# RL-VIG/LibContinual

Hardware: AMD Instinct MI355X
Metric: images/sec/node (task-0 epoch), CIFAR-100 B50-5x10 (higher is better)
Workload: dtype bf16; 1 GPU; lwf_resnet18_b50_task0; method=LWF, backbone=resnet18, per_gpu_batch=256, global_batch=256, image=3x32x32, parallelism=dp1, optimizer=fused SGD

## Files before the change

include/clhip.h:

```cpp
#ifndef CLHIP_H
#define CLHIP_H

#include <stddef.h>
#include <stdint.h>

#ifdef __cplusplus
extern "C" {
#endif

#define CLHIP_OK 0
#define CLHIP_EINVAL (-1)
#define CLHIP_EHIP (-2)
#define CLHIP_ENOMEM (-3)

#define CLHIP_BF16 0
#define CLHIP_F32 1

const char* clhip_last_error(void);
int clhip_version(void);

int clhip_nchw_to_nhwc(const float* x, void* y, int N, int C, int H, int W, int Cpad, int dtype, void* stream);
int clhip_nhwc_to_nchw(const void* y, float* x, int N, int C, int H, int W, int dtype, void* stream);

int clhip_conv_weight_prep(const float* w, void* w_fwd, void* w_dg, int K, int taps, int Creal, int Cpad,
// ... 225 lines not shown
    void* relu_mask;
} clhip_bn_res_input;
int clhip_conv_fwd_acc_bn_res_input(const void* z_in, const clhip_bn_input* bn , const clhip_bn_res_input* rs , const void* w_fwd, void* z,
                                    double* stat_acc, int replicas, int N, int H, int W, int C, int K, int ksize, int stride, int pad, int dtype,
                                    void* stream);
int clhip_conv_bn_input_wt_supported(int N, int H, int W, int C, int K, int ksize, int stride, int pad, int dtype);
int clhip_conv_fwd_acc_bn_input_wt(const void* z_in, const clhip_bn_input* bn , const clhip_bn_res_input* rs , const void* w_fwd, void* z,
                                   double* stat_acc, int replicas, int N, int H, int W, int C, int K, int ksize, int stride, int pad, int dtype,
                                   void* stream);
#define CLHIP_CONV_STEM7 1
#define CLHIP_CONV_STEM 2
#define CLHIP_CONV_CONV64 3
#define CLHIP_CONV_CONV16 4
#define CLHIP_CONV_CONV8 5
#define CLHIP_CONV_CONV5 6
#define CLHIP_CONV_CONV9 7
#define CLHIP_CONV_CONV4 8
#define CLHIP_CONV_CONV3 9
#define CLHIP_CONV_CONV2 10
#define CLHIP_CONV_V1 11
#define CLHIP_CONV_SHORTCUT 12
#define CLHIP_CONV_WGRAD_STEM7 13
#define CLHIP_CONV_WGRAD_STEM 14
#define CLHIP_CONV_WGRAD64 15
#define CLHIP_CONV_WGRAD4 16
#define CLHIP_CONV_WGRAD3 17
#define CLHIP_CONV_WGRAD16 18
#define CLHIP_CONV_WGRAD32 19
#define CLHIP_CONV_WGRAD2_DET 20
#define CLHIP_CONV_WGRAD2_ATOMIC 21
#define CLHIP_CONV_WGRAD_V1 22
#define CLHIP_CONV_WGRAD_V1_NO_TR 23
int clhip_conv_route(int op, int form, int N, int H, int W, int C, int Creal, int K, int ksize, int stride, int pad, int dtype);
int clhip_conv_dgrad_wgrad_bn_input(const void* x_z, const float* x_coef, const void* dz, const void* w_dg, void* dx, int accumulate, float* dw,
                                    void* ws, const float* mean, const float* invstd, double* acc , int replicas, int N, int H, int W,
                                    int C, int Creal, int K, int ksize, int stride, int pad, int dtype, void* stream);

int clhip_conv_dgrad_pair_supported(int N, int H, int W, int C, int K, int dtype);
size_t clhip_conv_dgrad_pair_packed_bytes(int C, int K);
int clhip_conv_dgrad_pair_pack(const void* w_dg, const void* w_sc_dg , void* packed, int C, int K, int dtype, void* stream);
int clhip_conv_dgrad_pair(const void* dz, const void* w_packed, const void* dz_sc , void* dx, int accumulate, int N, int H,
                          int W, int C, int K, int dtype, void* stream);

int clhip_conv_dgrad_pair_bn_reduce_supported(int N, int H, int W, int C, int K, int dtype);
int clhip_conv_dgrad_pair_bn_reduce(const void* dz, const void* w_packed, const void* dz_sc , void* dx, int accumulate, const void* z_prod,
                                    const void* y_prod , const float* mean, const float* invstd, double* acc, int replicas, int N, int H,
                                    int W, int C, int K, int dtype, void* stream);
int clhip_conv_wgrad_pair_supported(int N, int H, int W, int C, int K, int dtype);
int clhip_conv_fwd_acc_pair_supported(int N, int H, int W, int C, int K, int dtype);
int clhip_conv_fwd_acc_pair(const void* x, const void* w_fwd, const void* w_sc_fwd, void* z, void* z_sc, double* stat_acc, int replicas,
                            double* stat_acc_sc, int replicas_sc, int N, int H, int W, int C, int K, int dtype, void* stream);
int clhip_conv_wgrad_pair(const void* x, const void* dz, const void* dz_sc, float* dw, float* dw_sc, void* ws, void* ws_sc, int N, int H, int W,
                          int C, int K, int dtype, void* stream);

int clhip_config(const char* key, const char* value);
const char* clhip_config_get(const char* key);
void clhip_gemm8_config(int mode);
void clhip_wgrad4_config(int target_workgroups);
int clhip_attn_fwd(const void* qkv, void* out, float* lse, int B, int N, int H, int D, int dtype, void* stream);
int clhip_attn_bwd(const void* qkv, const void* out, const float* lse, const void* dout, void* dqkv, float* dsum_ws, int B, int N,
                   int H, int D, int dtype, void* stream);
int clhip_attn_prefix_fwd(const void* qkv, const void* pk, const void* pv, void* out, float* lse, int B, int N, int Lp, int H, int D, int dtype, void* stream);
int clhip_attn_prefix_bwd(const void* qkv, const void* pk, const void* pv, const void* out, const float* lse, const void* dout, void* dqkv, float* dpk,
                          float* dpv, float* dsum_ws, int B, int N, int Lp, int H, int D, int dtype, void* stream);
size_t clhip_coda_ws_bytes(int layers, int B, int s, int f);
int clhip_coda_fwd(int layers, const float* q, const float* const* K, const float* const* A, const float* const* P, void* const* ek, void* const* ev, float* c,
// ... 130 lines not shown
```

libcontinual_amd/_lib.py:

```python
import ctypes as C
import os
import re
import subprocess

_HERE = os.path.dirname(os.path.abspath(__file__))
LIB_PATH = os.path.join(_HERE, "libclhip.so")
HEADER_PATH = os.path.join(os.path.dirname(_HERE), "include", "clhip.h")

BF16, F32 = 0, 1
(CONV_STEM7, CONV_STEM, CONV_CONV64, CONV_CONV16, CONV_CONV8, CONV_CONV5, CONV_CONV9, CONV_CONV4, CONV_CONV3, CONV_CONV2, CONV_V1, CONV_SHORTCUT, CONV_WGRAD_STEM7,
 CONV_WGRAD_STEM, CONV_WGRAD64, CONV_WGRAD4, CONV_WGRAD3, CONV_WGRAD16, CONV_WGRAD32, CONV_WGRAD2_DET, CONV_WGRAD2_ATOMIC, CONV_WGRAD_V1, CONV_WGRAD_V1_NO_TR) = range(1, 24)


class ClhipError(RuntimeError):
    pass


class UnitDesc(C.Structure):
    _fields_ = [("cin", C.c_int32), ("cout", C.c_int32), ("ksize", C.c_int32), ("stride", C.c_int32), ("pad", C.c_int32),
                ("src", C.c_int32), ("res", C.c_int32), ("relu", C.c_int32),
                ("w_off", C.c_int64), ("gamma_off", C.c_int64), ("beta_off", C.c_int64),
                ("rm_off", C.c_int64), ("rv_off", C.c_int64)]


# ... 108 lines not shown
    "clhip_ce_slice": (_i, [_p, _p, _i, _i, _i, _i, _i, _f, _p, _i, _p, _i, _p, _p, _p]),
    "clhip_ce_window": (_i, [_p, _p, _i, _i, _i, _i, _i, _i, _f, _p, _i, _p, _i, _p, _p, _p]),
    "clhip_kd_loss": (_i, [_p, _i, _p, _i, _i, _i, _f, _f, _p, _i, _p, _i, _p]),
    "clhip_cosine_linear_fwd": (_i, [_p, _p, _p, _p, _p, _i, _i, _i, _p]),
    "clhip_cosine_linear_bwd": (_i, [_p, _p, _p, _p, _p, _p, _p, _p, _i, _i, _i, _i, _p]),
    "clhip_cos_embed_loss": (_i, [_p, _p, _i, _i, _f, _p, _i, _p, _i, _p]),
    "clhip_margin_rank_loss": (_i, [_p, _p, _i, _i, _i, _i, _f, _f, _p, _i, _p, _i, _p, _p]),
    "clhip_ewc_penalty": (_i, [_p, _p, _p, _l, _f, _p, _i, _p]),
    "clhip_ewc_grad": (_i, [_p, _p, _p, _p, _l, _f, _p, _p]),
    "clhip_ewc_penalty_multi": (_i, [_i, _p, _p, _p, _p, _f, _p, _i, _p]),
    "clhip_ewc_grad_multi": (_i, [_i, _p, _p, _p, _p, _p, _f, _p, _p]),
    "clhip_fisher_accum": (_i, [_p, _p, _l, _f, _p]),
    "clhip_fisher_merge": (_i, [_p, _p, _l, _f, _p]),
    "clhip_sgd_step": (_i, [_p, _p, _p, _l, _f, _f, _f, _f, _p, _p, _f, _p]),
    "clhip_sgd_step_multi": (_i, [_i, _p, _p, _p, _p, _f, _f, _f, _f, _p]),
    "clhip_sgd_step_multi_zero": (_i, [_i, _p, _p, _p, _p, _f, _f, _f, _f, C.c_uint, _p]),
    "clhip_adam_step": (_i, [_p, _p, _p, _p, _l, _f, _f, _f, _f, _f, _f, _i, _p]),
    "clhip_sq_norm": (_i, [_p, _l, _p, _i, _p]),
    "clhip_scale": (_i, [_p, _l, _f, _p]),
    "clhip_scale_dev": (_i, [_p, _p, _l, _f, _p, _p]),
    "clhip_sigma_scale_fwd": (_i, [_p, _p, _p, _l, _p]),
    "clhip_sigma_scale_bwd": (_i, [_p, _p, _p, _p, _p, _i, _l, _p]),
    "clhip_l2_normalize_rows": (_i, [_p, _p, _i, _i, _p]),
    "clhip_ncm_classify": (_i, [_p, _p, _i, _i, _i, _p, _p]),
    "clhip_herding_select": (_i, [_p, _i, _i, _i, _p, _p, _p]),
    "clhip_herding_select_batched": (_i, [_p, _p, _i, _i, _i, _i, _p, _p, _p]),
    "clhip_augment_crop_flip": (_i, [_p, _p, _p, _p, _p, _i, _i, _i, _i, _i, C.POINTER(C.c_float), C.POINTER(C.c_float), _p]),
    "clhip_augment_rrc_flip": (_i, [_p, _p, _p, _p, _i, _i, _i, _i, C.POINTER(C.c_float), C.POINTER(C.c_float), _p]),
    "clhip_augment_rrc_aa_ws_bytes": (_sz, [_i, _i, _i]),
    "clhip_augment_rrc_aa": (_i, [_p, _p, _p, _p, _p, _p, _p, _i, _i, _i, _i, _i, C.POINTER(C.c_float), C.POINTER(C.c_float), _p]),
    "clhip_gemm_nt": (_i, [_p, _p, _p, _p, _p, _p] + [_i] * 10 + [_p]),
    "clhip_gemm_nt_route": (_i, [_i] * 9 + [C.POINTER(C.c_int), _i]),
    "clhip_conv_route": (_i, [_i] * 12),
    "clhip_config": (_i, [C.c_char_p, C.c_char_p]),
    "clhip_config_get": (C.c_char_p, [C.c_char_p]),
    "clhip_conv_bn_input_wt_supported": (_i, [_i] * 9),
    "clhip_conv_fwd_acc_bn_input_wt": (_i, [_p, _p, _p, _p, _p, _p, _i] + [_i] * 9 + [_p]),
    "clhip_gram_accum_batched": (_i, [_p, C.c_size_t, _i, _p, _i, _i, _i, _p]),
    "clhip_gemm8_config": (None, [_i]),
    "clhip_wgrad4_config": (None, [_i]),
    "clhip_attn_fwd": (_i, [_p, _p, _p, _i, _i, _i, _i, _i, _p]),
    "clhip_attn_bwd": (_i, [_p, _p, _p, _p, _p, _p, _i, _i, _i, _i, _i, _p]),
    "clhip_attn_prefix_fwd": (_i, [_p, _p, _p, _p, _p, _i, _i, _i, _i, _i, _i, _p]),
    "clhip_attn_prefix_bwd": (_i, [_p] * 10 + [_i] * 6 + [_p]),
    "clhip_coda_ws_bytes": (_sz, [_i, _i, _i, _i]),
    "clhip_coda_fwd": (_i, [_i, _p, _p, _p, _p, _p, _p, _p, _i, _i, _i, _i, _i, _i, _p]),
    "clhip_coda_bwd": (_i, [_i] + [_p] * 11 + [_i] * 6 + [_p]),
    "clhip_dual_fwd": (_i, [_i, _i] + [_p] * 9 + [_i] * 8 + [_p]),
    "clhip_dual_bwd": (_i, [_i, _i] + [_p] * 8 + [_i] * 6 + [_p]),
    "clhip_ln_fwd": (_i, [_p, _p, _p, _p, _p, _p, _i, _i, _f, _i, _p]),
    "clhip_ln_bwd": (_i, [_p, _p, _p, _p, _p, _p, _i, _i, _i, _p]),
    "clhip_ln_pool_fwd": (_i, [_p, _p, _p, _p, _i, _i, _i, _i, _f, _i, _p]),
    "clhip_ln_pool_bwd": (_i, [_p, _p, _p, _p, _i, _i, _i, _i, _f, _i, _p]),
    "clhip_patchify": (_i, [_p, _p, _i, _i, _i, _i, _p]),
    "clhip_vit_assemble": (_i, [_p, _p, _p, _p, _p, _i, _i, _i, _i, _i, _p]),
    "clhip_vit_prompt_grad": (_i, [_p, _p, _i, _i, _i, _i, _i, _p]),
    "clhip_weight_prep2": (_i, [_p, _p, _p, _i, _i, _p, _p, _p, _p, _i, _i, _p]),
    "clhip_lora_qkv_refresh": (_i, [_i, _p, _p, _p, _p, _p, _p, _p, _i, _i, _i, _p]),
    "clhip_lora_merge": (_i, [_p, _p, _p, _p, _p, _i, _i, _p]),
    "clhip_lora_grad_ws_bytes": (_sz, [_i, _i, _i]),
    "clhip_lora_acat": (_i, [_p, _p, _p, _i, _i, _i, _p]),
    "clhip_lora_grad": (_i, [_p, _p, _p, _p, _p, _p, _p, _p, _i, _i, _i, _i, _p]),
    "clhip_gram_accum": (_i, [_p, _p, _i, _i, _i, _p]),
    "clhip_l2p_select": (_i, [_p, _p, _p, _i, _i, _i, _i, _i, _p, _p, _p, _p, _p, _p]),
    "clhip_l2p_scatter": (_i, [_p, _p, _p, _i, _i, _i, _i, _p]),
    "clhip_vit_create": (_p, [C.POINTER(VitDesc), _i]),
# ... 82 lines not shown
```

libcontinual_amd/csrc/api.hip:

```cpp
#include <map>
#include <utility>
#include <vector>
#include <mutex>
#include <string>
#include <string.h>
#include <stdio.h>
#include <stdlib.h>

#include "kernels.h"

static thread_local char g_err[512] = "";

void clhip_set_error(const char* fmt, ...) {
    va_list ap;
    va_start(ap, fmt);
    vsnprintf(g_err, sizeof(g_err), fmt, ap);
    va_end(ap);
}

extern "C" const char* clhip_last_error(void) { return g_err; }
extern "C" int clhip_version(void) { return 103; }

namespace {
const char* const kKeys[] = {
    "ATTN_GENERIC", "ATTN_BWD", "BN_FUSE", "BN_FUSE_MAX_M", "BN_MASK_BITS", "BN_MASK_FROM_Y", "BN_PARTIALS", "CE_ROWS", "CE_ONE_WG", "LINEAR_BWD_SPLIT", "CONV3G", "CONV4", "CONV_V1",
    "GEMM_NO_SPLIT", "GEMM_TAIL", "NO_CONV16", "NO_CONV3", "NO_PARITY_DGRAD", "NO_SHORTCUT", "NO_STEM", "PREP_NARROW", "WGRAD4",
    "WGRAD_NO_TR", "WGRAD2_ATOMIC", "WGRAD_DEFER", "WGRAD_DEFER_SIDE", "BWD_FUSED", "WGRAD_STREAM", "BRANCH_STREAM", "WGRAD_ALWAYS_QUEUE", "SIDE_PRIO", "EVENT_FLAGS", "EVENT_RECORD", "CONV5", "CONV6", "WGRAD16_PARTS", "WGRAD32_IPG", "WGRAD64_IPG", "WGRAD64_IPI2", "CONV64", "CONV64_BM", "CONV64_FWD", "CONV6_PAIR", "CONV7", "CONV7_TPW", "WGRAD7", "FWD7", "PAIR_BN_FUSE", "POOL_BN_FUSE", "BN_INPUT", "BN_INPUT_WT", "BN_RES_INPUT", "BN_GRAD", "BN_GRAD_MINC", "BN_GRAD_RES", "CONV6_DEBUG", "BN_ONEPASS", "WGRAD5", "WGRAD32",
    "BN_ACC_CPT", "BN_BWD_ITERS", "CONV3_CFG", "CONV4_CFG", "CONV4_GRID", "GEMM_GROUP_M", "GEMM_MT", "IGEMM_TILE",
    "SHORTCUT_MIN_PIXELS", "STEM_GRID", "STEM_WGRAD_GRID", "WGRAD4_MIN_STEPS", "WGRAD4_MIN_TOTAL", "WGRAD_NET_GFLOP", "WGRAD_TARGET",
    "CONV5_MIN_TILES", "CONV5_GRID", "CONV64_MAX_W", "CONV64_MAX_M", "CONV8", "CONV8_MIN_TILES", "DZ_BUFFERS", "CONV8_GRID", "CONV8_OPT", "CONV8_BNR", "CONV9", "PLAN_SKIP", "WT_DEBUG", "EVAL_LAZY", "GEMM_SPLITK", "STREAM_PROBE", "STAGE_EVAL", "STAGE_TRAIN", "STAGE_TRAIN_BWD", "STAGE_TRACE", "STAGE_ENTRY", "STAGE_ENTRY_BWD", "STAGE_POOL", "STAGE_XCH3", "ADAPTER_TM",
    "CONV3_DEBUG", "WGRAD_DEBUG", "CONV4_FORCE_CFG", "CONV4_ENABLE", "CONV4_DEBUG", "CONV4_TRACE", "WGRAD4_TRACE", "CONV6_TRACE", "CONV8_TRACE", "CONV9_TRACE",
};
std::mutex g_stream_mu;
std::mutex g_cfg_mu;
std::map<std::string, const char*>& cfg_map() { static std::map<std::string, const char*> m; return m; }
bool known_key(const char* k) {
    for (const char* q : kKeys) if (strcmp(q, k) == 0) return true;
    return false;
}
}

namespace {
__global__ void stream_probe_spin_kernel(unsigned long long* out, long long ticks) {
    const unsigned long long t0 = wall_clock64();
    while ((long long)(wall_clock64() - t0) < ticks) __builtin_amdgcn_s_sleep(64);
    out[0] = wall_clock64();
}
__global__ void stream_probe_stamp_kernel(unsigned long long* out) { out[1] = wall_clock64(); }

struct SharedStreams {
    std::vector<hipStream_t> pool;
    std::map<std::pair<hipStream_t, int>, hipStream_t> chosen;
    hipStream_t low_prio = nullptr;
    unsigned long long* probe_buf = nullptr;
};
SharedStreams g_shared[16];

bool runs_beside(SharedStreams& S, hipStream_t a, hipStream_t b) {
// ... 111 lines not shown
```

libcontinual_amd/csrc/bn.hip:

```cpp
#include <stdlib.h>

#include <hip/hip_ext.h>

#include "kernels.h"

namespace {

__global__ __launch_bounds__(256) void bn_finalize_kernel(const float* __restrict__ part, int tiles, double invM, double unbias,
                                                          int C, const float* __restrict__ gamma, const float* __restrict__ beta,
                                                          float* rm, float* rv, float momentum, float eps, float* mean_o,
                                                          float* invstd_o, float* scale, float* shift) {
    const int lane = threadIdx.x & 63, wave = threadIdx.x >> 6;
    const int c = blockIdx.x * 4 + wave;
    if (c >= C) return;
    double s1 = 0.0, s2 = 0.0;
    for (int t = lane; t < tiles; t += 64) {
        s1 += (double)part[((size_t)t * 2 + 0) * C + c];
        s2 += (double)part[((size_t)t * 2 + 1) * C + c];
    }
#pragma unroll
    for (int o = 32; o > 0; o >>= 1) { s1 += __shfl_xor(s1, o, 64); s2 += __shfl_xor(s2, o, 64); }
    if (lane == 0) {
        double mean = s1 * invM;
        double var = s2 * invM - mean * mean;
// ... 193 lines not shown
}

template <typename T, bool RELU, int DRES>
__global__ __launch_bounds__(256) void bn_bwd_apply_kernel(const T* __restrict__ dy, const T* __restrict__ y,
                                                           const T* __restrict__ z, const float* __restrict__ mean,
                                                           const float* __restrict__ invstd, const float* __restrict__ gamma,
                                                           const float* __restrict__ coef, T* __restrict__ dz, T* __restrict__ dres,
                                                           int64_t nchunks, int C) {
    const int64_t stride = (int64_t)gridDim.x * blockDim.x;
    for (int64_t i = (int64_t)blockIdx.x * blockDim.x + threadIdx.x; i < nchunks; i += stride) {
        const int c0 = (int)((i * 8) % C);
        float g[8], yy[8], zz[8], o[8], rr[8];
        load8<T>(dy + i * 8, g);
        load8<T>(z + i * 8, zz);
        if (RELU) load8<T>(y + i * 8, yy);
        if (DRES == 2) load8<T>(dres + i * 8, rr);
#pragma unroll
        for (int e = 0; e < 8; ++e) {
            const int c = c0 + e;
            float gg = g[e];
            if (RELU) gg = yy[e] > 0.f ? gg : 0.f;
            const float is = invstd[c];
            const float xh = (zz[e] - mean[c]) * is;
            o[e] = gamma[c] * is * (gg - coef[c] - xh * coef[C + c]);
            g[e] = gg;
            if (DRES == 2) rr[e] += gg;
        }
        store8<T>(dz + i * 8, o);
        if (DRES == 1) store8<T>(dres + i * 8, g);
        if (DRES == 2) store8<T>(dres + i * 8, rr);
    }
}

template <typename T, bool RES, bool RELU>
__global__ __launch_bounds__(256) void bn_apply_train_kernel(const T* __restrict__ z, const double* __restrict__ acc, int rep, double invM, double unbias,
                                                             const float* __restrict__ gamma, const float* __restrict__ beta, float* rm, float* rv,
                                                             float momentum, float eps, float* __restrict__ mean_o, float* __restrict__ invstd_o,
                                                             const T* __restrict__ res, T* __restrict__ y, int64_t nchunks, int C,
                                                             unsigned char* __restrict__ relu_mask = nullptr) {
    extern __shared__ __attribute__((aligned(16))) float coefs[];
    __shared__ double sred[256];
    const bool narrow = 2 * C <= 128;
    if (narrow) replica_parts(acc, rep, C, sred);
    for (int c = threadIdx.x; c < C; c += 256) {
        const bool upd = blockIdx.x == 0 && rm != nullptr;
        const float rm_old = upd ? rm[c] : 0.f, rv_old = upd ? rv[c] : 0.f;
        double s1 = 0.0, s2 = 0.0;
        if (narrow) { for (int q = 0; q < 256 / (2 * C); ++q) { s1 += sred[q * 2 * C + c]; s2 += sred[q * 2 * C + C + c]; } }
        else sum_strided2(acc + c, acc + C + c, rep, 2 * (size_t)C, s1, s2);
        const double mean = s1 * invM;
        double var = s2 * invM - mean * mean;
        if (var < 0.0) var = 0.0;
        float istd;
        if constexpr (sizeof(T) == 4) istd = (float)(1.0 / sqrt(var + (double)eps));
        else istd = rsqrtf((float)var + eps);
        const float sc = gamma[c] * istd;
        coefs[c] = sc;
        coefs[C + c] = beta[c] - (float)mean * sc;
        if (blockIdx.x == 0) {
            mean_o[c] = (float)mean;
            invstd_o[c] = istd;
            if (rm != nullptr) {
                rm[c] = (1.f - momentum) * rm_old + momentum * (float)mean;
                rv[c] = (1.f - momentum) * rv_old + momentum * (float)(var * unbias);
            }
        }
    }
    __syncthreads();
    const int64_t stride = (int64_t)gridDim.x * blockDim.x;
    const int64_t i0 = (int64_t)blockIdx.x * blockDim.x + threadIdx.x;
    const int c0 = ((int)i0 & ((C >> 3) - 1)) * 8;
    float sc[8], sh[8];
#pragma unroll
    for (int e = 0; e < 8; ++e) { sc[e] = coefs[c0 + e]; sh[e] = coefs[C + c0 + e]; }
    constexpr int UN = 4;
    for (int64_t i = i0; i < nchunks; i += stride * UN) {
        float v[UN][8], r[UN][8];
#pragma unroll
        for (int u = 0; u < UN; ++u) {
            const int64_t iu = i + u * stride;
            if (iu < nchunks) { load8<T>(z + iu * 8, v[u]); if (RES) load8<T>(res + iu * 8, r[u]); }
        }
#pragma unroll
        for (int u = 0; u < UN; ++u) {
            const int64_t iu = i + u * stride;
            if (iu >= nchunks) break;
#pragma unroll
            for (int e = 0; e < 8; ++e) {
                float o = fmaf(v[u][e], sc[e], sh[e]);
                if (RES) o += r[u][e];
                if (RELU) o = fmaxf(o, 0.f);
                v[u][e] = o;
            }
            store8<T>(y + iu * 8, v[u]);
            if (RELU && relu_mask != nullptr) {
                unsigned m = 0;
#pragma unroll
                for (int e = 0; e < 8; ++e) m |= (stored_positive<T>(v[u][e]) ? 1u : 0u) << e;
                relu_mask[iu] = (unsigned char)m;
            }
        }
    }
}

template <typename T, int RELU, int DRES>
__global__ __launch_bounds__(256) void bn_bwd_apply_acc_kernel(const T* __restrict__ dy, const T* __restrict__ y, const T* __restrict__ z,
                                                               const float* __restrict__ mean, const float* __restrict__ invstd,
                                                               const float* __restrict__ gamma, const double* __restrict__ acc, int rep, double invM,
                                                               float* dgamma, float* dbeta, T* __restrict__ dz, T* __restrict__ dres,
                                                               int64_t nchunks, int C, const float* __restrict__ beta = nullptr) {
    extern __shared__ __attribute__((aligned(16))) float coefs[];
    __shared__ double sred[256];
    const bool narrow = 2 * C <= 128;
    if (narrow) replica_parts(acc, rep, C, sred);
    for (int c = threadIdx.x; c < C; c += 256) {
        const float db_old = blockIdx.x == 0 ? dbeta[c] : 0.f, dg_old = blockIdx.x == 0 ? dgamma[c] : 0.f;
        const float m = mean[c], is_c = invstd[c], gi_c = gamma[c] * is_c;
        const float sh_c = RELU == 2 ? beta[c] - m * gi_c : 0.f;
        double s1 = 0.0, s2 = 0.0;
        if (narrow) { for (int q = 0; q < 256 / (2 * C); ++q) { s1 += sred[q * 2 * C + c]; s2 += sred[q * 2 * C + C + c]; } }
        else sum_strided2(acc + c, acc + C + c, rep, 2 * (size_t)C, s1, s2);
        coefs[c] = (float)(s1 * invM);
        coefs[C + c] = (float)(s2 * invM);
        coefs[2 * C + c] = m;
        coefs[3 * C + c] = is_c;
        coefs[4 * C + c] = gi_c;
        coefs[5 * C + c] = sh_c;
        if (blockIdx.x == 0) { dbeta[c] = db_old + (float)s1; dgamma[c] = dg_old + (float)s2; }
    }
    __syncthreads();
    const int64_t stride = (int64_t)gridDim.x * blockDim.x;
    const int64_t i0 = (int64_t)blockIdx.x * blockDim.x + threadIdx.x;
    const int c0 = ((int)i0 & ((C >> 3) - 1)) * 8;
    float k0[8], k1[8], gi[8], mu[8], is[8], sh[8];
#pragma unroll
    for (int e = 0; e < 8; ++e) {
        k0[e] = coefs[c0 + e];
        k1[e] = coefs[C + c0 + e];
        mu[e] = coefs[2 * C + c0 + e];
        is[e] = coefs[3 * C + c0 + e];
        gi[e] = coefs[4 * C + c0 + e];
        if (RELU == 2) sh[e] = coefs[5 * C + c0 + e];
    }
    constexpr int UN = sizeof(T) == 2 ? 4 : 2;
    for (int64_t i = i0; i < nchunks; i += stride * UN) {
        float g[UN][8], yy[UN][8], zz[UN][8], rr[UN][8];
        unsigned mk[UN];
#pragma unroll
        for (int u = 0; u < UN; ++u) {
            mk[u] = 0;
            const int64_t iu = i + u * stride;
            if (iu < nchunks) {
                load8<T>(dy + iu * 8, g[u]);
                load8<T>(z + iu * 8, zz[u]);
                if (RELU == 1) load8<T>(y + iu * 8, yy[u]);
                if (RELU == 3) mk[u] = reinterpret_cast<const unsigned char*>(y)[iu];
                if (DRES == 2) load8<T>(dres + iu * 8, rr[u]);
            }
        }
#pragma unroll
        for (int u = 0; u < UN; ++u) {
            const int64_t iu = i + u * stride;
            if (iu >= nchunks) break;
            float o[8];
#pragma unroll
            for (int e = 0; e < 8; ++e) {
                float gg = g[u][e];
                if (RELU == 1) gg = yy[u][e] > 0.f ? gg : 0.f;
                if (RELU == 2) gg = stored_positive<T>(fmaf(zz[u][e], gi[e], sh[e])) ? gg : 0.f;
                if (RELU == 3) gg = (mk[u] >> e) & 1u ? gg : 0.f;
                const float xh = (zz[u][e] - mu[e]) * is[e];
                o[e] = gi[e] * (gg - k0[e] - xh * k1[e]);
                g[u][e] = gg;
                if (DRES == 2) rr[u][e] += gg;
            }
            store8<T>(dz + iu * 8, o);
            if (DRES == 1) store8<T>(dres + iu * 8, g[u]);
            if (DRES == 2) store8<T>(dres + iu * 8, rr[u]);
        }
    }
}

int bn_bwd_blocks(int64_t M, int C) {
    int cpr = C >> 3;
    int rpi = 256 / cpr;
    int64_t g = (M + rpi - 1) / rpi;
    static const int forced = clhip_cfg("BN_BWD_ITERS") ? atoi(clhip_cfg("BN_BWD_ITERS")) : 0;
    int64_t iters = forced > 0 ? forced : g / 128;
    if (iters < 1) iters = 1;
    if (iters > 8) iters = 8;
    g = (g + iters - 1) / iters;
    if (g > 1024) g = 1024;
    if (g < 1) g = 1;
    return (int)g;
}

// ... 586 lines not shown
```

libcontinual_amd/csrc/conv2.hip:

```cpp
#include <stdlib.h>

#include "kernels.h"

namespace {

constexpr int BK2 = 64;

struct ConvParams2 {
    const void* src;
    const void* wt;
    void* dst;
    float* stats;
    double* stat_acc;
    int stat_rep;
    int N, Hs, Ws, Cs, log2Cs, Hd, Wd, Cd, ksize, stride, pad, accumulate;
    int M, K;
    int cls_tiles;
};

template <typename T> struct Chunk2;
template <> struct Chunk2<bf16_t> { uint4 a; };
template <> struct Chunk2<float> { uint4 a, b; };

template <typename T> __device__ __forceinline__ Chunk2<T> zero2() {
    Chunk2<T> c;
    if constexpr (sizeof(T) == 2) { c.a = make_uint4(0, 0, 0, 0); }
    else { c.a = make_uint4(0, 0, 0, 0); c.b = make_uint4(0, 0, 0, 0); }
    return c;
}
template <typename T> __device__ __forceinline__ Chunk2<T> gload2(const T* p) {
    Chunk2<T> c;
    if constexpr (sizeof(T) == 2) { c.a = *reinterpret_cast<const uint4*>(p); }
    else { c.a = *reinterpret_cast<const uint4*>(p); c.b = *reinterpret_cast<const uint4*>(p + 4); }
// ... 290 lines not shown
    dim3 grid((p.M + BM - 1) / BM, (p.Cd + BN - 1) / BN);
    ConvParams2 q = p;
    if (q.cls_tiles > 0) {
        q.cls_tiles = (q.M / 4 + BM - 1) / BM;
        grid.x = 4 * q.cls_tiles;
    }
    hipLaunchKernelGGL(kern, grid, dim3(256), lds, st, q);
    CLHIP_LAUNCH_CHECK();
    return CLHIP_OK;
}

template <typename T, int MODE>
int launch2(const ConvParams2& p, hipStream_t st) {
    TileCfg t = pick_tile(p.cls_tiles > 0 ? p.M / 4 : p.M, p.Cd);
    if (t.bn == 128) {
        if (t.bm == 128) return launch_cfg<T, 2, 2, 4, 4, MODE>(p, st);
        return launch_cfg<T, 1, 4, 4, 2, MODE>(p, st);
    }
    if (t.bn == 64) {
        if (t.bm == 256) return launch_cfg<T, 4, 1, 4, 4, MODE>(p, st);
        if (t.bm == 128) return launch_cfg<T, 4, 1, 2, 4, MODE>(p, st);
        return launch_cfg<T, 4, 1, 1, 4, MODE>(p, st);
    }
    if (t.bn == 32) {
        if (t.bm == 256) return launch_cfg<T, 4, 1, 4, 2, MODE>(p, st);
        if (t.bm == 128) return launch_cfg<T, 4, 1, 2, 2, MODE>(p, st);
        return launch_cfg<T, 4, 1, 1, 2, MODE>(p, st);
    }
    if (t.bm == 256) return launch_cfg<T, 4, 1, 4, 1, MODE>(p, st);
    if (t.bm == 128) return launch_cfg<T, 4, 1, 2, 1, MODE>(p, st);
    return launch_cfg<T, 4, 1, 1, 1, MODE>(p, st);
}

}

int clhip_conv2_tiles_m(int M, int Cd) { return (M + pick_tile(M, Cd).bm - 1) / pick_tile(M, Cd).bm; }

int clhip_conv2_launch(const void* src, const void* wt, void* dst, float* stats, double* stat_acc, int stat_rep, int N, int Hs, int Ws, int Cs, int Hd, int Wd,
                       int Cd, int ksize, int stride, int pad, int accumulate, int mode, int dtype, hipStream_t st) {
    ConvParams2 p;
    p.src = src; p.wt = wt; p.dst = dst; p.stats = stats; p.stat_acc = stat_acc; p.stat_rep = stat_rep > 0 ? stat_rep : 1;
    p.N = N; p.Hs = Hs; p.Ws = Ws; p.Cs = Cs; p.log2Cs = ilog2_exact(Cs); p.Hd = Hd; p.Wd = Wd; p.Cd = Cd;
    p.ksize = ksize; p.stride = stride; p.pad = pad; p.accumulate = accumulate;
    p.M = N * Hd * Wd; p.K = ksize * ksize * Cs;
    static const bool nocls = clhip_cfg("NO_PARITY_DGRAD") != nullptr;
    p.cls_tiles = (!nocls && mode == 1 && stride == 2 && ksize == 3 && Cs >= 32 && p.log2Cs >= 0 && (Hd % 2 == 0) && (Wd % 2 == 0)) ? 1 : 0;
    if (dtype == CLHIP_BF16) return mode == 0 ? launch2<bf16_t, 0>(p, st) : launch2<bf16_t, 1>(p, st);
    return mode == 0 ? launch2<float, 0>(p, st) : launch2<float, 1>(p, st);
}

namespace {

#ifdef CLHIP_ABLATION
#define DBGW2(p) ((p).debug)
#else
#define DBGW2(p) 0
#endif

struct WgradParams2 {
    const void* x; const void* dz; float* dw;
    int N, H, W, C, log2C, Creal, Ho, Wo, lgHo, lgWo, K, ksize, stride, pad;
    int M, J, pix_per_split, debug;
    float* slab;
    int64_t slab_stride;
};

template <typename T>
__device__ __forceinline__ Chunk2<T> lds_ld_tr(const char* tile, int pitch, int pix0, int col0, int lane) {
    const int fr = lane & 15, fg = lane >> 4;
    Chunk2<T> c;
    if constexpr (sizeof(T) == 2) {
        const char* a0 = tile + (pix0 + fg * 8 + (fr >> 2)) * pitch + (col0 + (fr & 3) * 4) * 2;
// ... 219 lines not shown
```

libcontinual_amd/trainer.py:

```python
import copy
import os
import sys
from time import time

import numpy as np
import torch
from torch.utils.data import DataLoader

from . import ops, parallel
from . import scheduler as sched
from .utils import AverageMeter, compute_bwt, compute_frgt, count_all_parameters, count_parameters, get_instance, init_seed, quiesce_gc

_OBSERVE_DOES_BACKWARD = ("L2P",)


_UNIT_GRADS = {}


def _backward(loss):
    if loss.is_cuda and loss.dim() == 0 and loss.dtype == torch.float32:
        one = _UNIT_GRADS.get(loss.device)
        if one is None:
            one = _UNIT_GRADS[loss.device] = torch.ones((), device=loss.device, dtype=torch.float32)
            ops.UNIT_GRAD_PTRS.add(one.data_ptr())
        torch.autograd.backward(loss, grad_tensors=one)
    else:
        loss.backward()


class GraphedStep:
    WARM, KEEP = 2, 4
    PROBE = 12
    _PLAN_SWITCHES = (b"BN_INPUT", b"BN_INPUT_WT", b"BN_RES_INPUT", b"BN_GRAD", b"BN_GRAD_RES", b"BN_FUSE", b"BRANCH_STREAM", b"WGRAD_STREAM", b"CONV6_PAIR",
                      b"STAGE_EVAL", b"EVAL_LAZY", b"STAGE_TRAIN", b"STAGE_TRAIN_BWD", b"STAGE_ENTRY", b"STAGE_POOL", b"STAGE_XCH3", b"GEMM8", b"GEMM_TAIL", b"ATTN_BWD")

    def __init__(self, model, optimizer, method_name, reducer=None):
        self.model, self.optimizer, self.method_name = model, optimizer, method_name
        self.reducer = reducer
        from .optim import _owner_of
        owners = {}
        for group in optimizer.param_groups:
            for p in group["params"]:
                o = _owner_of(p)
                if o is not None:
                    owners[id(o)] = o
        self.owners = list(owners.values())
        self.graphs = {}
        self.seen = {}
        self.stream = torch.cuda.Stream()
        self.choice = {}
        self._probe = {}
        self.disabled = False
        self.fallback_ok = True

    def _key(self, batch):
        shapes = tuple((k, tuple(v.shape), str(v.dtype)) for k, v in sorted(batch.items()) if torch.is_tensor(v))
        lrs = tuple((g.get("lr"), g.get("momentum"), g.get("weight_decay")) for g in self.optimizer.param_groups)
        from . import _lib
        L = _lib.lib()
        cfg = tuple(L.clhip_config_get(k) for k in self._PLAN_SWITCHES)
        red = self.reducer
        dp = None if red is None else (red.world, red.exchange, getattr(self.optimizer, "grad_scale", None))
        return shapes, lrs, self.model.training, cfg, dp

    def _step(self, batch):
        if self.method_name in _OBSERVE_DOES_BACKWARD:
            self.optimizer.zero_grad()
# ... 496 lines not shown
```

Before: 131,400 images/sec.

## Add pipelined LDS-direct stride-2 entry conv kernel and prefetch BN apply loads

Adds a specialized bf16 3x3 stride-2 downsampling convolution kernel for stage-entry layers. It uses buffer loads straight into LDS with a three-stage ring, MFMA accumulation and fused BN statistics, and is enabled by default under an ENTRY_S2 switch that is also registered as a plan switch. It also issues the first global loads in the BN apply forward and backward kernels before the coefficient reduction and syncthreads, so memory latency overlaps the reduction. The cost is extra register pressure and one more kernel variant; a launch counter is exported for observability.

```diff
diff --git a/include/clhip.h b/include/clhip.h
--- a/include/clhip.h
+++ b/include/clhip.h
@@ -281,6 +281,7 @@
 #define CLHIP_CONV_WGRAD_V1 22
 #define CLHIP_CONV_WGRAD_V1_NO_TR 23
 int clhip_conv_route(int op, int form, int N, int H, int W, int C, int Creal, int K, int ksize, int stride, int pad, int dtype);
+long long clhip_conv_entry_s2_launches(void);
 int clhip_conv_dgrad_wgrad_bn_input(const void* x_z, const float* x_coef, const void* dz, const void* w_dg, void* dx, int accumulate, float* dw,
                                     void* ws, const float* mean, const float* invstd, double* acc , int replicas, int N, int H, int W,
                                     int C, int Creal, int K, int ksize, int stride, int pad, int dtype, void* stream);
diff --git a/libcontinual_amd/_lib.py b/libcontinual_amd/_lib.py
--- a/libcontinual_amd/_lib.py
+++ b/libcontinual_amd/_lib.py
@@ -164,6 +164,7 @@
     "clhip_gemm_nt": (_i, [_p, _p, _p, _p, _p, _p] + [_i] * 10 + [_p]),
     "clhip_gemm_nt_route": (_i, [_i] * 9 + [C.POINTER(C.c_int), _i]),
     "clhip_conv_route": (_i, [_i] * 12),
+    "clhip_conv_entry_s2_launches": (C.c_longlong, []),
     "clhip_config": (_i, [C.c_char_p, C.c_char_p]),
     "clhip_config_get": (C.c_char_p, [C.c_char_p]),
     "clhip_conv_bn_input_wt_supported": (_i, [_i] * 9),
diff --git a/libcontinual_amd/csrc/api.hip b/libcontinual_amd/csrc/api.hip
--- a/libcontinual_amd/csrc/api.hip
+++ b/libcontinual_amd/csrc/api.hip
@@ -23,7 +23,7 @@
 
 namespace {
 const char* const kKeys[] = {
-    "ATTN_GENERIC", "ATTN_BWD", "BN_FUSE", "BN_FUSE_MAX_M", "BN_MASK_BITS", "BN_MASK_FROM_Y", "BN_PARTIALS", "CE_ROWS", "CE_ONE_WG", "LINEAR_BWD_SPLIT", "CONV3G", "CONV4", "CONV_V1",
+    "ATTN_GENERIC", "ATTN_BWD", "BN_FUSE", "BN_FUSE_MAX_M", "BN_MASK_BITS", "BN_MASK_FROM_Y", "BN_PARTIALS", "CE_ROWS", "CE_ONE_WG", "LINEAR_BWD_SPLIT", "CONV3G", "CONV4", "CONV_V1", "ENTRY_S2",
     "GEMM_NO_SPLIT", "GEMM_TAIL", "NO_CONV16", "NO_CONV3", "NO_PARITY_DGRAD", "NO_SHORTCUT", "NO_STEM", "PREP_NARROW", "WGRAD4",
     "WGRAD_NO_TR", "WGRAD2_ATOMIC", "WGRAD_DEFER", "WGRAD_DEFER_SIDE", "BWD_FUSED", "WGRAD_STREAM", "BRANCH_STREAM", "WGRAD_ALWAYS_QUEUE", "SIDE_PRIO", "EVENT_FLAGS", "EVENT_RECORD", "CONV5", "CONV6", "WGRAD16_PARTS", "WGRAD32_IPG", "WGRAD64_IPG", "WGRAD64_IPI2", "CONV64", "CONV64_BM", "CONV64_FWD", "CONV6_PAIR", "CONV7", "CONV7_TPW", "WGRAD7", "FWD7", "PAIR_BN_FUSE", "POOL_BN_FUSE", "BN_INPUT", "BN_INPUT_WT", "BN_RES_INPUT", "BN_GRAD", "BN_GRAD_MINC", "BN_GRAD_RES", "CONV6_DEBUG", "BN_ONEPASS", "WGRAD5", "WGRAD32",
     "BN_ACC_CPT", "BN_BWD_ITERS", "CONV3_CFG", "CONV4_CFG", "CONV4_GRID", "GEMM_GROUP_M", "GEMM_MT", "IGEMM_TILE",
diff --git a/libcontinual_amd/csrc/bn.hip b/libcontinual_amd/csrc/bn.hip
--- a/libcontinual_amd/csrc/bn.hip
+++ b/libcontinual_amd/csrc/bn.hip
@@ -249,6 +249,20 @@
     }
 }
 
+template <typename T> struct Raw8;
+template <> struct Raw8<bf16_t> { uint4 a; };
+template <> struct Raw8<float> { float4 a, b; };
+template <typename T> __device__ __forceinline__ Raw8<T> raw_load8(const T* p) {
+    Raw8<T> r;
+    if constexpr (sizeof(T) == 2) { r.a = *reinterpret_cast<const uint4*>(p); }
+    else { r.a = *reinterpret_cast<const float4*>(p); r.b = *reinterpret_cast<const float4*>(p + 4); }
+    return r;
+}
+template <typename T> __device__ __forceinline__ void raw_unpack8(const Raw8<T>& r, float (&v)[8]) {
+    if constexpr (sizeof(T) == 2) { unpack8(r.a, v); }
+    else { v[0] = r.a.x; v[1] = r.a.y; v[2] = r.a.z; v[3] = r.a.w; v[4] = r.b.x; v[5] = r.b.y; v[6] = r.b.z; v[7] = r.b.w; }
+}
+
 template <typename T, bool RES, bool RELU>
 __global__ __launch_bounds__(256) void bn_apply_train_kernel(const T* __restrict__ z, const double* __restrict__ acc, int rep, double invM, double unbias,
                                                              const float* __restrict__ gamma, const float* __restrict__ beta, float* rm, float* rv,
@@ -256,6 +270,15 @@
                                                              const T* __restrict__ res, T* __restrict__ y, int64_t nchunks, int C,
                                                              unsigned char* __restrict__ relu_mask = nullptr) {
     extern __shared__ __attribute__((aligned(16))) float coefs[];
+    constexpr int UN = 4;
+    const int64_t stride = (int64_t)gridDim.x * blockDim.x;
+    const int64_t i0 = (int64_t)blockIdx.x * blockDim.x + threadIdx.x;
+    Raw8<T> pv[UN], pr[UN];
+#pragma unroll
+    for (int u = 0; u < UN; ++u) {
+        const int64_t iu = i0 + u * stride;
+        if (iu < nchunks) { pv[u] = raw_load8<T>(z + iu * 8); if (RES) pr[u] = raw_load8<T>(res + iu * 8); }
+    }
     __shared__ double sred[256];
     const bool narrow = 2 * C <= 128;
     if (narrow) replica_parts(acc, rep, C, sred);
@@ -284,24 +307,25 @@
         }
     }
     __syncthreads();
-    const int64_t stride = (int64_t)gridDim.x * blockDim.x;
-    const int64_t i0 = (int64_t)blockIdx.x * blockDim.x + threadIdx.x;
     const int c0 = ((int)i0 & ((C >> 3) - 1)) * 8;
     float sc[8], sh[8];
 #pragma unroll
     for (int e = 0; e < 8; ++e) { sc[e] = coefs[c0 + e]; sh[e] = coefs[C + c0 + e]; }
-    constexpr int UN = 4;
     for (int64_t i = i0; i < nchunks; i += stride * UN) {
         float v[UN][8], r[UN][8];
-#pragma unroll
-        for (int u = 0; u < UN; ++u) {
-            const int64_t iu = i + u * stride;
-            if (iu < nchunks) { load8<T>(z + iu * 8, v[u]); if (RES) load8<T>(res + iu * 8, r[u]); }
+        if (i != i0) {
+#pragma unroll
+            for (int u = 0; u < UN; ++u) {
+                const int64_t iu = i + u * stride;
+                if (iu < nchunks) { pv[u] = raw_load8<T>(z + iu * 8); if (RES) pr[u] = raw_load8<T>(res + iu * 8); }
+            }
         }
 #pragma unroll
         for (int u = 0; u < UN; ++u) {
             const int64_t iu = i + u * stride;
             if (iu >= nchunks) break;
+            raw_unpack8<T>(pv[u], v[u]);
+            if (RES) raw_unpack8<T>(pr[u], r[u]);
 #pragma unroll
             for (int e = 0; e < 8; ++e) {
                 float o = fmaf(v[u][e], sc[e], sh[e]);
@@ -327,6 +351,26 @@
                                                                float* dgamma, float* dbeta, T* __restrict__ dz, T* __restrict__ dres,
                                                                int64_t nchunks, int C, const float* __restrict__ beta = nullptr) {
     extern __shared__ __attribute__((aligned(16))) float coefs[];
+    constexpr int UN = sizeof(T) == 2 ? 4 : 2;
+    const int64_t stride = (int64_t)gridDim.x * blockDim.x;
+    const int64_t i0 = (int64_t)blockIdx.x * blockDim.x + threadIdx.x;
+    Raw8<T> pg[UN], pz[UN], py[UN], pr[UN];
+    unsigned mk[UN];
+    auto issue = [&](int64_t i) {
+#pragma unroll
+        for (int u = 0; u < UN; ++u) {
+            mk[u] = 0;
+            const int64_t iu = i + u * stride;
+            if (iu < nchunks) {
+                pg[u] = raw_load8<T>(dy + iu * 8);
+                pz[u] = raw_load8<T>(z + iu * 8);
+                if (RELU == 1) py[u] = raw_load8<T>(y + iu * 8);
+                if (RELU == 3) mk[u] = reinterpret_cast<const unsigned char*>(y)[iu];
+                if (DRES == 2) pr[u] = raw_load8<T>(dres + iu * 8);
+            }
+        }
+    };
+    issue(i0);
     __shared__ double sred[256];
     const bool narrow = 2 * C <= 128;
     if (narrow) replica_parts(acc, rep, C, sred);
@@ -346,8 +390,6 @@
         if (blockIdx.x == 0) { dbeta[c] = db_old + (float)s1; dgamma[c] = dg_old + (float)s2; }
     }
     __syncthreads();
-    const int64_t stride = (int64_t)gridDim.x * blockDim.x;
-    const int64_t i0 = (int64_t)blockIdx.x * blockDim.x + threadIdx.x;
     const int c0 = ((int)i0 & ((C >> 3) - 1)) * 8;
     float k0[8], k1[8], gi[8], mu[8], is[8], sh[8];
 #pragma unroll
@@ -359,26 +401,17 @@
         gi[e] = coefs[4 * C + c0 + e];
         if (RELU == 2) sh[e] = coefs[5 * C + c0 + e];
     }
-    constexpr int UN = sizeof(T) == 2 ? 4 : 2;
     for (int64_t i = i0; i < nchunks; i += stride * UN) {
         float g[UN][8], yy[UN][8], zz[UN][8], rr[UN][8];
-        unsigned mk[UN];
-#pragma unroll
-        for (int u = 0; u < UN; ++u) {
-            mk[u] = 0;
-            const int64_t iu = i + u * stride;
-            if (iu < nchunks) {
-                load8<T>(dy + iu * 8, g[u]);
-                load8<T>(z + iu * 8, zz[u]);
-                if (RELU == 1) load8<T>(y + iu * 8, yy[u]);
-                if (RELU == 3) mk[u] = reinterpret_cast<const unsigned char*>(y)[iu];
-                if (DRES == 2) load8<T>(dres + iu * 8, rr[u]);
-            }
-        }
+        if (i != i0) issue(i);
 #pragma unroll
         for (int u = 0; u < UN; ++u) {
             const int64_t iu = i + u * stride;
             if (iu >= nchunks) break;
+            raw_unpack8<T>(pg[u], g[u]);
+            raw_unpack8<T>(pz[u], zz[u]);
+            if (RELU == 1) raw_unpack8<T>(py[u], yy[u]);
+            if (DRES == 2) raw_unpack8<T>(pr[u], rr[u]);
             float o[8];
 #pragma unroll
             for (int e = 0; e < 8; ++e) {
diff --git a/libcontinual_amd/csrc/conv2.hip b/libcontinual_amd/csrc/conv2.hip
--- a/libcontinual_amd/csrc/conv2.hip
+++ b/libcontinual_amd/csrc/conv2.hip
@@ -1,4 +1,6 @@
 #include <stdlib.h>
+
+#include <atomic>
 
 #include "kernels.h"
 
@@ -355,12 +357,234 @@
     return launch_cfg<T, 4, 1, 1, 1, MODE>(p, st);
 }
 
-}
+typedef __attribute__((address_space(3))) void lvoid_t;
+
+std::atomic<unsigned long long> g_entry_s2_launches{0};
+
+struct EntryS2Params {
+    const bf16_t* src;
+    const bf16_t* wt;
+    bf16_t* dst;
+    float* stats;
+    double* stat_acc;
+    int stat_rep;
+    int N, H, W, Cs, Cd, Hd, Wd, M;
+    int lgWd, lgHd, cpt_shift;
+};
+
+constexpr int ES_NST = 3;
+
+template <int N> __device__ __forceinline__ void es_wait_vm() { __builtin_amdgcn_s_waitcnt((N & 15) | 0x70 | 0xF00 | ((N >> 4) << 14)); }
+__device__ __forceinline__ void es_barrier() {
+    __builtin_amdgcn_s_waitcnt(0xC07F);
+    __builtin_amdgcn_s_barrier();
+    asm volatile("" ::: "memory");
+}
+
+template <int WM, int WN, int MT, int NT>
+__global__ __launch_bounds__(256) void conv_entry_s2_kernel(const EntryS2Params p) {
+    typedef bf16_t T;
+    constexpr int BM = WM * MT * 16, BN = WN * NT * 16;
+    constexpr int A_BYTES = BM * 128, STAGE = (BM + BN) * 128;
+    constexpr int AINST = BM / 8 / 4, BINST = BN / 8 / 4, WINST = AINST + BINST;
+    static_assert(WM * WN == 4 && AINST >= 1 && BINST >= 1 && AINST * 32 == BM && BINST * 32 == BN, "ring rows must divide among the four waves");
+    extern __shared__ __attribute__((aligned(16))) char smem[];
+    const int tid = threadIdx.x, lane = tid & 63;
+    const int wave = __builtin_amdgcn_readfirstlane(tid >> 6);
+    const int wm = wave / WN, wn = wave % WN;
+    const int m0 = blockIdx.x * BM, n0 = blockIdx.y * BN;
+    const int Cs = p.Cs, W = p.W, K9 = 9 * Cs;
+    constexpr int OOB = 0x40000000;
+
+    const int drow = lane >> 3, dslot = lane & 7;
+    int aoff[AINST], boff[BINST];
+    unsigned amask[AINST];
+#pragma unroll
+    for (int i = 0; i < AINST; ++i) {
+        const int row = (wave * AINST + i) * 8 + drow, pix = m0 + row;
+        aoff[i] = 0; amask[i] = 0;
+        if (pix < p.M) {
+            const int wo = pix & (p.Wd - 1), t = pix >> p.lgWd, ho = t & (p.Hd - 1), n = t >> p.lgHd;
+            const int h0 = 2 * ho - 1, w0 = 2 * wo - 1;
+            aoff[i] = (((n * p.H + h0) * W + w0) * Cs) * 2 + ((dslot ^ drow) << 4);
+            unsigned m = 0;
+#pragma unroll
+            for (int r = 0; r < 3; ++r)
+#pragma unroll
+                for (int s = 0; s < 3; ++s)
+                    if ((unsigned)(h0 + r) < (unsigned)p.H && (unsigned)(w0 + s) < (unsigned)W) m |= 1u << (3 * r + s);
+            amask[i] = m;
+        }
+    }
+#pragma unroll
+    for (int i = 0; i < BINST; ++i) {
+        const int row = (wave * BINST + i) * 8 + drow;
+        boff[i] = ((n0 + row) * K9) * 2 + ((dslot ^ drow) << 4);
+    }
+    const __amdgpu_buffer_rsrc_t srs = __builtin_amdgcn_make_buffer_rsrc(const_cast<bf16_t*>(p.src), 0, p.N * p.H * W * Cs * 2, 0x00020000);
+    const __amdgpu_buffer_rsrc_t wrs = __builtin_amdgcn_make_buffer_rsrc(const_cast<bf16_t*>(p.wt), 0, p.Cd * K9 * 2, 0x00020000);
+    auto issue = [&](int k, int stage) {
+        const int tap = k >> p.cpt_shift, chunk = k - (tap << p.cpt_shift);
+        const int r = tap / 3, s = tap - 3 * r;
+        const int tapoff = ((r * W + s) * Cs + chunk * 64) * 2;
+        const unsigned bit = 1u << tap;
+        char* l = smem + stage * STAGE;
+#if defined(__HIP_DEVICE_COMPILE__)
+#pragma unroll
+        for (int i = 0; i < AINST; ++i)
+            __builtin_amdgcn_raw_ptr_buffer_load_lds(srs, (lvoid_t*)(l + (wave * AINST + i) * 1024), 16, (amask[i] & bit) ? aoff[i] + tapoff : OOB, 0, 0, 0);
+#pragma unroll
+        for (int i = 0; i < BINST; ++i)
+            __builtin_amdgcn_raw_ptr_buffer_load_lds(wrs, (lvoid_t*)(l + A_BYTES + (wave * BINST + i) * 1024), 16, boff[i] + k * 128, 0, 0, 0);
+#else
+        (void)tapoff; (void)bit; (void)l;
+#endif
+    };
+
+    f32x4 acc[MT][NT];
+#pragma unroll
+    for (int i = 0; i < MT; ++i)
+#pragma unroll
+        for (int j = 0; j < NT; ++j) acc[i][j] = f32x4{0.f, 0.f, 0.f, 0.f};
+
+    const int fr = lane & 15, fg = lane >> 4;
+    const int nk = 9 << p.cpt_shift;
+    issue(0, 0);
+    issue(1, 1);
+#pragma unroll 1
+    for (int k0 = 0; k0 < nk; k0 += 3) {
+#pragma unroll
+        for (int s3 = 0; s3 < 3; ++s3) {
+            const int k = k0 + s3;
+            if (k + 1 < nk) es_wait_vm<WINST>(); else es_wait_vm<0>();
+            es_barrier();
+            if (k + 2 < nk) issue(k + 2, (s3 + 2) % 3);
+            const char* As = smem + s3 * STAGE;
+            const char* Bs = As + A_BYTES;
+#pragma unroll
+            for (int ks = 0; ks < 2; ++ks) {
+                bf16x8_t xf[MT], wf[NT];
+#pragma unroll
+                for (int i = 0; i < MT; ++i) xf[i] = *reinterpret_cast<const bf16x8_t*>(As + lds_off2<T>((wm * MT + i) * 16 + fr, ks * 4 + fg));
+#pragma unroll
+                for (int j = 0; j < NT; ++j) wf[j] = *reinterpret_cast<const bf16x8_t*>(Bs + lds_off2<T>((wn * NT + j) * 16 + fr, ks * 4 + fg));
+#pragma unroll
+                for (int i = 0; i < MT; ++i)
+#pragma unroll
+                    for (int j = 0; j < NT; ++j) acc[i][j] = __builtin_amdgcn_mfma_f32_16x16x32_bf16(wf[j], xf[i], acc[i][j], 0, 0, 0);
+            }
+        }
+    }
+
+#pragma unroll
+    for (int i = 0; i < MT; ++i) {
+        const int pix = m0 + (wm * MT + i) * 16 + fr;
+        if (pix < p.M) {
+#pragma unroll
+            for (int j = 0; j < NT; ++j) {
+                const int o = n0 + (wn * NT + j) * 16 + fg * 4;
+                uint2 u;
+                u.x = pack_bf16x2(acc[i][j][0], acc[i][j][1]);
+                u.y = pack_bf16x2(acc[i][j][2], acc[i][j][3]);
+                *reinterpret_cast<uint2*>(p.dst + (size_t)pix * p.Cd + o) = u;
+            }
+        }
+    }
+    if (p.stats == nullptr && p.stat_acc == nullptr) return;
+
+    es_barrier();
+    float* red = reinterpret_cast<float*>(smem);
+    float sv[8 * NT];
+#pragma unroll
+    for (int j = 0; j < NT; ++j)
+#pragma unroll
+        for (int e = 0; e < 4; ++e) {
+            float s1 = 0.f, s2 = 0.f;
+#pragma unroll
+            for (int i = 0; i < MT; ++i) { const float v = acc[i][j][e]; s1 += v; s2 = fmaf(v, v, s2); }
+            sv[j * 4 + e] = s1;
+            sv[4 * NT + j * 4 + e] = s2;
+        }
+    row16_sum_n(sv);
+    if (fr == 0) {
+#pragma unroll
+        for (int j = 0; j < NT; ++j) {
+            const int c = (wn * NT + j) * 16 + fg * 4;
+            *reinterpret_cast<float4*>(red + (wm * 2 + 0) * BN + c) = make_float4(sv[j * 4], sv[j * 4 + 1], sv[j * 4 + 2], sv[j * 4 + 3]);
+            *reinterpret_cast<float4*>(red + (wm * 2 + 1) * BN + c) = make_float4(sv[4 * NT + j * 4], sv[4 * NT + j * 4 + 1], sv[4 * NT + j * 4 + 2], sv[4 * NT + j * 4 + 3]);
+        }
+    }
+    es_barrier();
+    for (int idx = tid; idx < 2 * BN; idx += 256) {
+        const int which = idx / BN, c = idx - which * BN;
+        float t = 0.f;
+#pragma unroll
+        for (int w = 0; w < WM; ++w) t += red[(w * 2 + which) * BN + c];
+        if (p.stat_acc != nullptr) atomicAdd(p.stat_acc + ((size_t)(blockIdx.x & (p.stat_rep - 1)) * 2 + which) * p.Cd + n0 + c, (double)t);
+        else p.stats[((size_t)blockIdx.x * 2 + which) * p.Cd + n0 + c] = t;
+    }
+}
+
+bool entry_s2_domain(const void* stats, const double* stat_acc, int N, int Hs, int Ws, int Cs, int Hd, int Wd, int Cd, int ksize, int stride, int pad,
+                     int accumulate, int mode, int dtype) {
+    if (!(mode == 0 && dtype == CLHIP_BF16 && !(stats != nullptr && stat_acc != nullptr) && accumulate == 0)) return false;
+    if (!(ksize == 3 && stride == 2 && pad == 1 && Cd == 2 * Cs && (Cs == 64 || Cs == 128 || Cs == 256))) return false;
+    if (!(Hs == Ws && (Hs == 8 || Hs == 16 || Hs == 32) && Hd == Hs / 2 && Wd == Ws / 2 && N >= 1)) return false;
+    return (int64_t)N * Hs * Ws * Cs * 2 < ((int64_t)1 << 29);
+}
+
+template <int WM, int WN, int MT, int NT>
+int launch_entry_s2_cfg(const EntryS2Params& p, hipStream_t st) {
+    constexpr int BM = WM * MT * 16, BN = WN * NT * 16;
+    constexpr size_t lds = (size_t)ES_NST * (BM + BN) * 128;
+    static_assert(lds <= 160 * 1024 && lds >= WM * 2 * BN * sizeof(float), "LDS of one CU; the statistics scratch aliases the ring");
+    auto kern = conv_entry_s2_kernel<WM, WN, MT, NT>;
+    int dev = 0;
+    (void)hipGetDevice(&dev);
+    static bool attr_set[16] = {false};
+    if (dev < 0 || dev >= 16 || !attr_set[dev]) {
+        if (hipFuncSetAttribute(reinterpret_cast<const void*>(kern), hipFuncAttributeMaxDynamicSharedMemorySize, (int)lds) != hipSuccess) {
+            clhip_set_error("conv2 entry body: cannot reserve %zu bytes of LDS", lds);
+            return CLHIP_EHIP;
+        }
+        if (dev >= 0 && dev < 16) attr_set[dev] = true;
+    }
+    hipLaunchKernelGGL(kern, dim3((p.M + BM - 1) / BM, p.Cd / BN), dim3(256), lds, st, p);
+    CLHIP_LAUNCH_CHECK();
+    g_entry_s2_launches.fetch_add(1, std::memory_order_relaxed);
+    return CLHIP_OK;
+}
+
+int launch_entry_s2(const void* src, const void* wt, void* dst, float* stats, double* stat_acc, int stat_rep, int N, int Hs, int Ws, int Cs, int Hd, int Wd, int Cd,
+                    hipStream_t st, bool* launched) {
+    *launched = false;
+    const TileCfg t = pick_tile(N * Hd * Wd, Cd);
+    if (t.bn != 128 || t.bm != 64) return CLHIP_OK;
+    EntryS2Params p;
+    p.src = static_cast<const bf16_t*>(src); p.wt = static_cast<const bf16_t*>(wt); p.dst = static_cast<bf16_t*>(dst);
+    p.stats = stats; p.stat_acc = stat_acc; p.stat_rep = stat_rep > 0 ? stat_rep : 1;
+    p.N = N; p.H = Hs; p.W = Ws; p.Cs = Cs; p.Cd = Cd; p.Hd = Hd; p.Wd = Wd; p.M = N * Hd * Wd;
+    p.lgWd = ilog2_exact(Wd); p.lgHd = ilog2_exact(Hd); p.cpt_shift = ilog2_exact(Cs / 64);
+    *launched = true;
+    return launch_entry_s2_cfg<1, 4, 4, 2>(p, st);
+}
+
+}
+
+extern "C" long long clhip_conv_entry_s2_launches(void) { return (long long)g_entry_s2_launches.load(std::memory_order_relaxed); }
 
 int clhip_conv2_tiles_m(int M, int Cd) { return (M + pick_tile(M, Cd).bm - 1) / pick_tile(M, Cd).bm; }
 
 int clhip_conv2_launch(const void* src, const void* wt, void* dst, float* stats, double* stat_acc, int stat_rep, int N, int Hs, int Ws, int Cs, int Hd, int Wd,
                        int Cd, int ksize, int stride, int pad, int accumulate, int mode, int dtype, hipStream_t st) {
+    if (entry_s2_domain(stats, stat_acc, N, Hs, Ws, Cs, Hd, Wd, Cd, ksize, stride, pad, accumulate, mode, dtype)) {
+        const char* sw = clhip_cfg("ENTRY_S2");
+        if (sw == nullptr || atoi(sw) != 0) {
+            bool launched = false;
+            const int rc = launch_entry_s2(src, wt, dst, stats, stat_acc, stat_rep, N, Hs, Ws, Cs, Hd, Wd, Cd, st, &launched);
+            if (launched || rc != CLHIP_OK) return rc;
+        }
+    }
     ConvParams2 p;
     p.src = src; p.wt = wt; p.dst = dst; p.stats = stats; p.stat_acc = stat_acc; p.stat_rep = stat_rep > 0 ? stat_rep : 1;
     p.N = N; p.Hs = Hs; p.Ws = Ws; p.Cs = Cs; p.log2Cs = ilog2_exact(Cs); p.Hd = Hd; p.Wd = Wd; p.Cd = Cd;
diff --git a/libcontinual_amd/trainer.py b/libcontinual_amd/trainer.py
--- a/libcontinual_amd/trainer.py
+++ b/libcontinual_amd/trainer.py
@@ -32,7 +32,7 @@
     WARM, KEEP = 2, 4
     PROBE = 12
     _PLAN_SWITCHES = (b"BN_INPUT", b"BN_INPUT_WT", b"BN_RES_INPUT", b"BN_GRAD", b"BN_GRAD_RES", b"BN_FUSE", b"BRANCH_STREAM", b"WGRAD_STREAM", b"CONV6_PAIR",
-                      b"STAGE_EVAL", b"EVAL_LAZY", b"STAGE_TRAIN", b"STAGE_TRAIN_BWD", b"STAGE_ENTRY", b"STAGE_POOL", b"STAGE_XCH3", b"GEMM8", b"GEMM_TAIL", b"ATTN_BWD")
+                      b"STAGE_EVAL", b"EVAL_LAZY", b"STAGE_TRAIN", b"STAGE_TRAIN_BWD", b"STAGE_ENTRY", b"STAGE_POOL", b"STAGE_XCH3", b"GEMM8", b"GEMM_TAIL", b"ATTN_BWD", b"ENTRY_S2")
 
     def __init__(self, model, optimizer, method_name, reducer=None):
         self.model, self.optimizer, self.method_name = model, optimizer, method_name
```

New measurement: 134,900 images/sec (median of 6 runs). 2.7% higher.
